# ZencashOfficial/ginger-lib

Hardware: AMD Instinct MI355X
Metric: MNT4-753 G1 MSM scalar-muls/sec + 2^n NTT ms at 1/2/4/8 MI355X (higher is better)
Workload: dtype u32 (29-bit limbs of 753-bit Montgomery residues, 64-bit accumulators)

## Files before the change

ginger-lib_amd/asmgen/build.py:

```python
import json
import os
import subprocess
import sys

from . import g1_reduce, g1_xyzz, g2_rounds, microbench, ntt_pass
from .isa import module_text

LLVM = os.environ.get("GH_LLVM_BIN", "/opt/rocm/lib/llvm/bin")

P4 = 0x1c4c62d92c41110229022eee2cdadb7f997505b8fafed5eb7e8f96c97d87307fdb925e8a0ed8d99d124d9a15af79db117e776f218059db80f0da5cb537e38685acce9767254a4638810719ac425f0e39d54522cdd119f5e9063de245e8001
P6 = 0x1c4c62d92c41110229022eee2cdadb7f997505b8fafed5eb7e8f96c97d87307fdb925e8a0ed8d99d124d9a15af79db26c5c28c859a99b3eebca9429212636b9dff97634993aa4d6c381bc3f0057974ea099170fa13a4fd90776e240000001
R = 1 << 754


def programs():
    progs = [
        g1_xyzz.build("gh_asm_acc_g1_p4", P4, R % P4),
        g1_xyzz.build("gh_asm_acc_g1_p6", P6, R % P6),
        g1_xyzz.build("gh_asm_acc_g1_p4_pw", P4, R % P4, persistent=True),
        g1_xyzz.build("gh_asm_acc_g1_p6_pw", P6, R % P6, persistent=True),
        g1_reduce.build("gh_asm_red_g1_p4", P4, R % P4),
        g1_reduce.build("gh_asm_red_g1_p6", P6, R % P6),
    ]
    c2 = g2_rounds.Cfg(2, 13, P4, R % P4)
# ... 6 lines not shown
                progs.append(g2_rounds.build("gh_asm_aff_%s_%s_%s" % (tag, "fwd" if fwd else "bwd", "r0" if r0 else "rn"), cfg, fwd, r0))
    for tag, prime in (("p4", P4), ("p6", P6)):
        for k in (6, 7, 8):
            progs.append(ntt_pass.build("gh_asm_ntt_%s_k%d" % (tag, k), prime, k))
    progs.append(microbench.build("gh_asm_mb_mulpair", P4))
    if os.environ.get("GH_ASM_DEBUG"):
        progs.append(g2_rounds.build("gh_asm_aff_f2_bwd_r0_dbg", c2, False, True, debug=True))
        for tag, prime in (("p4", P4), ("p6", P6)):
            progs.append(g1_xyzz.build("gh_asm_acc_g1_%s_dbg" % tag, prime, R % prime, debug=True))
            progs.append(g1_xyzz.build("gh_asm_acc_g1_%s_pw_dbg" % tag, prime, R % prime, persistent=True, debug=True))
    if os.environ.get("GH_ASM_VARIANTS"):
        progs += [g1_xyzz.build("gh_asm_acc_g1_p4_s1", P4, R % P4, split=1),
                  g1_xyzz.build("gh_asm_acc_g1_p4_s2", P4, R % P4, split=2),
                  g1_xyzz.build("gh_asm_acc_g1_p4_s1pf", P4, R % P4, split=1, prefetch=True)]
    return progs


def build(outdir):
    os.makedirs(outdir, exist_ok=True)
    progs = programs()
    text, infos = module_text(progs)
    s_path = os.path.join(outdir, "gh_asm.s")
    with open(s_path, "w") as f:
        f.write(text)
    o_path = os.path.join(outdir, "gh_asm.o")
    co_path = os.path.join(outdir, "gh_asm.hsaco")
    subprocess.run([os.path.join(LLVM, "clang"), "-x", "assembler", "-target", "amdgcn-amd-amdhsa", "-mcpu=gfx950",
                    "-c", s_path, "-o", o_path], check=True)
    subprocess.run([os.path.join(LLVM, "ld.lld"), "-shared", o_path, "-o", co_path], check=True)
    for p in progs:
        infos[p.name]["instructions"] = p.count()
        infos[p.name]["lds_bytes"] = p.lds_bytes
        infos[p.name]["scratch_bytes_per_lane"] = 0
    with open(os.path.join(outdir, "gh_asm.json"), "w") as f:
        json.dump(infos, f, indent=1, sort_keys=True)
    return co_path, infos


if __name__ == "__main__":
    co, infos = build(sys.argv[1] if len(sys.argv) > 1 else "build")
    print(co, json.dumps(infos))
```

ginger-lib_amd/asmgen/field.py:

```python
from .isa import Reg, V, S

NL = 26
LB = 29
LM = (1 << LB) - 1


def limbs(x, n=NL):
    return [(x >> (LB * i)) & LM for i in range(n)]


def unlimbs(l):
    return sum(int(v) << (LB * i) for i, v in enumerate(l))


class Chain:

    def __init__(self, acc, t0, t1, sdum, scar):
        self.acc = acc
        self.t0 = t0
        self.t1 = t1
        self.sdum = sdum
        self.scar = scar


class FieldGen:
    def __init__(self, prog, p, s_p, s_np, s_inv, s_lm):
        self.g = prog
        self.p = p
        self.pl = limbs(p)
        self.inv = (-pow(p, -1, 1 << LB)) % (1 << LB)
        self.s_p = s_p
        self.s_np = s_np
        self.s_inv = s_inv
        self.s_lm = s_lm

    def sP(self, i):
        return S(self.s_p + i)
# ... 227 lines not shown
                g.v_add3_u32(u, t, self.sNP(i), bw); yield
            g.v_ashrrev_i32(bw, LB, u); yield
            g.v_and_b32(b.sub(i), S(self.s_lm), u); yield
        g.v_cmp_eq_u32(ch.scar, 0, bw); yield
        for i in range(NL):
            g.v_cndmask_b32(a.sub(i), a.sub(i), b.sub(i), ch.scar); yield

    def neg_sel(self, ch, y, tmp, sel):
        g = self.g
        m, t0, lmm, x, c = ch.t1, ch.t0, ch.acc.lo(), ch.acc.hi(), tmp
        g.v_cndmask_b32(m, 0, -1, sel); yield
        g.v_and_b32(lmm, S(self.s_lm), m); yield
        g.v_and_b32(c, 1, m); yield
        for i in range(NL):
            g.v_and_b32(t0, self.sP(i), m); yield
            g.v_xor_b32(x, y.sub(i), lmm); yield
            g.v_add3_u32(x, x, t0, c); yield
            g.v_lshrrev_b32(c, LB, x); yield
            g.v_and_b32(y.sub(i), S(self.s_lm), x); yield

    def is_zero_mask(self, ch, a, smask):
        g = self.g
        t = ch.t0
        g.v_or3_b32(t, a.sub(0), a.sub(1), a.sub(2)); yield
        i = 3
        while i < NL:
            if i + 1 < NL:
                g.v_or3_b32(t, t, a.sub(i), a.sub(i + 1)); i += 2
            else:
                g.v_or_b32(t, t, a.sub(i)); i += 1
            yield
        g.v_cmp_eq_u32(smask, 0, t); yield

    def set_const(self, slot, value):
        for i, l in enumerate(limbs(value)):
            self.g.v_mov_b32(slot.sub(i), l)
            yield

    def copy(self, dst, src):
        for i in range(NL):
            self.g.v_mov_b32(dst.sub(i), src.sub(i))
            yield


def run(gen):
    for _ in gen:
        pass


def interleave(*gens):
    gens = list(gens)
    while gens:
        for g in list(gens):
            try:
                next(g)
            except StopIteration:
                gens.remove(g)
```

ginger-lib_amd/asmgen/g1_xyzz.py:

```python
from .isa import Prog, V, S, VCC, EXEC, OFF, fix_hazards
from .field import FieldGen, Chain, interleave, run, NL, LM

AFF_BYTES = 2 * NL * 4
PROJ_WORDS = 3 * NL
PARK_X, PARK_V, PARK_RR = 0, 1, 2
LDS_BYTES = 3 * NL * 256 * 4

S_KARG = S(0, 2)
S_WG = S(2)
S_BASES, S_SORTED, S_TASKS, S_SALTS = S(4, 2), S(6, 2), S(8, 2), S(10, 2)
S_NTASKS = S(12)
S_208 = S(13)
S_LM, S_INV = 20, 21
S_P, S_NP = 24, 50
S_ACTIVE = S(76, 2)
S_NEGSEL = S(78, 2)
S_T0, S_T1 = S(80, 2), S(82, 2)
S_LAUNCH = S(84, 2)
S_SAVE = S(86, 2)
S_DETOUR = S(88, 2)
S_T2 = S(90, 2)
S_ZERO = S(92, 2)
S_CTR = S(96, 2)
S_NTILES = S(98)
S_TILE = S(99)
S_BUDGET = S(3)
S_STAMPS = S(100, 2)
STAMP_BYTES = 64

V_TID, V_LDS = V(0), V(1)
V_CUR = V(2, 2)
V_LEFT, V_PHASE, V_SNEG, V_SALT = V(4), V(5), V(6), V(7)
V_DST = V(8, 2)
V_ADDR = V(10, 2)
# ... 9 lines not shown
V_ST0, V_ST1, V_STID, V_STOFF = V(30, 4), V(34, 4), V(26, 4), V(38)


def slot(i):
    return V(40 + NL * i, NL)


def seq(*gens):
    for gen in gens:
        run(gen)


E = [slot(i) for i in range(8)]


def build(name, p, one_mont, prefetch=False, split=4, persistent=False, debug=False):
    assert not (debug and prefetch)
    g = Prog(name)
    lanes = 64 if persistent else 256
    park_stride = lanes * 4
    g.lds_bytes = 3 * NL * park_stride
    for _ in range(4):
        g.add_arg(8, "ptr")
    g.add_arg(4, "val")
    if persistent:
        g.add_arg(4, "val")
        off_ctr = g.add_arg(8, "ptr")
        off_budget = g.add_arg(4, "val")
    if debug:
        off_stamps = g.add_arg(8, "ptr")
    f = FieldGen(g, p, S_P, S_NP, S_INV, S_LM)
    chA = Chain(V(248, 2), V(252), V(253), S(14, 2), S(16, 2))
    chB = Chain(V(250, 2), V(254), V(255), S(18, 2), S(22, 2))

    def park_addr(which, w):
        if which < 2:
            return V_LDS, (which * NL + w) * park_stride
        return V_LDS2, ((which - 2) * NL + w) * park_stride

    def park_put(which, sl):
        for w in range(NL):
            a, off = park_addr(which, w)
            g.ds_write_b32(a, sl.sub(w), offset=off)

    def park_get(which, sl):
        for w in range(NL):
            a, off = park_addr(which, w)
            g.ds_read_b32(sl.sub(w), a, offset=off)

    L_LOOP, L_INIT, L_INIT_RET, L_DETOUR, L_DET_RET, L_ADV, L_DONE, L_START = (
        g.uniq(s) for s in ("loop", "init", "init_ret", "detour", "det_ret", "adv", "done", "start"))
    S_JMP = S(94, 2)

    def stamp(dst):
        g.s_memtime(S_T0)
        g.s_memrealtime(S_T1)
        g.s_waitcnt(lgkmcnt=0)
        g.v_mov_b32(dst.sub(0), S_T0.lo()); g.v_mov_b32(dst.sub(1), S_T0.hi())
        g.v_mov_b32(dst.sub(2), S_T1.lo()); g.v_mov_b32(dst.sub(3), S_T1.hi())

    def stamp_store():
        stamp(V_ST1)
        g.s_getreg_b32(S_T0.lo(), "hwreg(HW_REG_HW_ID)")
        g.s_getreg_b32(S_T0.hi(), "hwreg(HW_REG_XCC_ID)")
        g.v_mov_b32(V_STID.sub(0), S_T0.lo()); g.v_mov_b32(V_STID.sub(1), S_T0.hi())
        g.v_mov_b32(V_STID.sub(3), S_LAUNCH.lo())
# ... 48 lines not shown
            g.v_lshrrev_b32(V_STID.sub(2), 6, V_T[0])
            g.v_lshlrev_b32(V_STOFF, 6, V_STID.sub(2))
        reset_task(V_T[0], with_constants=True)
        g.s_branch(L_LOOP)
    else:
        g.s_waitcnt(lgkmcnt=0)
        wave_constants()
        g.label(L_FETCH)
        g.s_mov_b64(EXEC, 1)
        g.v_mov_b32(V_T[0], 1)
        g.v_mov_b32(V_T[1], 0)
        g.global_atomic_add(V_T[2], V_T[1], V_T[0], S_CTR, sc0=True)
        g.s_waitcnt(vmcnt=0)
        g.v_readfirstlane_b32(S_TILE, V_T[2])
        g.s_mov_b64(EXEC, -1)
        g.s_cmp_ge_u32(S_TILE, S_NTILES)
        g.s_cbranch_scc1(L_EXIT)
        g.v_lshl_or_b32(V_T[0], S_TILE, 6, V_TID)
        g.v_cmp_gt_u32(VCC, S_NTASKS, V_T[0])
        g.s_and_b64(EXEC, EXEC, VCC)
        g.s_cbranch_execz(L_FETCH)
        g.s_mov_b64(S_LAUNCH, EXEC)
        if debug:
            stamp(V_ST0)
            g.v_mov_b32(V_STID.sub(2), S_TILE)
            g.v_lshlrev_b32(V_STOFF, 6, V_STID.sub(2))
        reset_task(V_T[0])
        g.s_branch(L_LOOP)
        g.label(L_EXIT)
        g.s_endpgm()

    g.label(L_DONE)
    g.s_mov_b64(EXEC, S_LAUNCH)
    run(f.is_zero_mask(chA, E[0], S_ZERO))
    park_get(PARK_X, E[2])
    park_get(PARK_V, E[3])
    g.v_cmp_ne_u32(S_NEGSEL, 0, V_SNEG)
    g.s_waitcnt(lgkmcnt=0)
    for w in range(NL):
        g.v_and_b32(E[2].sub(w), S(S_LM), E[2].sub(w))
        g.v_and_b32(E[3].sub(w), S(S_LM), E[3].sub(w))
    run(f.neg_sel(chA, E[3], V_TMP, S_NEGSEL))
    seq(f.mul(chA, E[2], E[1], E[4], E[2]),
        f.mul(chB, E[3], E[0], E[5], E[3]))
    run(f.cond_sub(chA, E[0], E[6], E[0]))
    run(f.mul(chA, E[0], E[1], E[6], E[2]))
    g.s_mov_b64(S_SAVE, EXEC)
    g.s_and_b64(EXEC, EXEC, S_ZERO)
    for w in range(NL):
        g.v_mov_b32(E[4].sub(w), 0)
        g.v_mov_b32(E[6].sub(w), 0)
    run(f.set_const(E[5], one_mont))
    g.s_mov_b64(EXEC, S_SAVE)
    for j in range(PROJ_WORDS // 2):
        g.global_store_dwordx2(V_DST, V(E[4].idx + 2 * j, 2), OFF, offset=8 * j)
    if debug:
        stamp_store()
    if persistent:
        g.s_sub_u32(S_BUDGET, S_BUDGET, 1)
        g.s_cmp_eq_u32(S_BUDGET, 0)
        g.s_cbranch_scc0(L_FETCH)
        g.s_endpgm()
    else:
        g.s_endpgm()

    g.label(L_LOOP)
    g.s_mov_b64(EXEC, S_LAUNCH)
    g.v_cmp_ne_u32(S_ACTIVE, 0, V_LEFT)
    g.v_cmp_ne_u32(S_T0, 0, V_GUARD)
    g.s_and_b64(S_ACTIVE, S_ACTIVE, S_T0)
    g.s_mov_b64(S_DETOUR, 0)
    g.s_and_b64(EXEC, S_ACTIVE, EXEC)
    g.s_cbranch_execz(L_DONE)
    g.global_load_dword(V_E, V_CUR, OFF)
    if prefetch:
        g.v_cmp_lt_u32(S_T1, 1, V_LEFT)
        g.v_cndmask_b32(V_T[2], 0, 4, S_T1)
        g.v_add_co_u32(V_NADDR.lo(), VCC, V_CUR.lo(), V_T[2])
        g.v_addc_co_u32(V_NADDR.hi(), VCC, 0, V_CUR.hi(), VCC)
        g.global_load_dword(V_ENEXT, V_NADDR, OFF)
    g.v_and_b32(V_T[1], 1, V_PHASE)
    g.v_cmp_ne_u32(S_T0, 0, V_T[1])
    g.v_mad_u64_u32(V(16, 2), chA.sdum, V_SALT, S_208, V_SALTS)
    g.s_waitcnt(vmcnt=0)
    g.v_and_b32(V_T[0], 0x7FFFFFFF, V_E)
    g.v_mad_u64_u32(V_ADDR, chA.sdum, V_T[0], S_208, V_BASES)
    g.v_cndmask_b32(V_ADDR.lo(), V_ADDR.lo(), V(16), S_T0)
    g.v_cndmask_b32(V_ADDR.hi(), V_ADDR.hi(), V(17), S_T0)
    if split > 1:
        g.s_mov_b64(S_SAVE, EXEC)
    for q in range(split):
        if split > 1:
            g.s_bfm_b64(S_T1, 64 // split, (64 // split) * q)
            g.s_and_b64(EXEC, S_SAVE, S_T1)
        for j in range(AFF_BYTES // 16):
            g.global_load_dwordx4(V(E[2].idx + 4 * j, 4), V_ADDR, OFF, offset=16 * j)
    if split > 1:
        g.s_mov_b64(EXEC, S_SAVE)
    g.v_lshrrev_b32(V_T[0], 31, V_E)
    g.v_lshrrev_b32(V_T[1], 1, V_PHASE)
    g.v_cndmask_b32(V_T[0], V_T[0], V_T[1], S_T0)
    g.v_xor_b32(V_T[0], V_T[0], V_SNEG)
    g.v_cmp_ne_u32(S_NEGSEL, 0, V_T[0])
    g.s_waitcnt(vmcnt=0)
    if prefetch:
        g.v_and_b32(V_T[2], 0x7FFFFFFF, V_ENEXT)
        g.v_mad_u64_u32(V_NADDR, chA.sdum, V_T[2], S_208, V_BASES)
        for j in range(4):
            g.global_load_dword(V_TOUCH, V_NADDR, OFF, offset=min(64 * j, AFF_BYTES - 4))
    run(f.neg_sel(chA, E[3], V_TMP, S_NEGSEL))
    run(f.is_zero_mask(chA, E[0], S_ZERO))
    g.s_cmp_lg_u64(S_ZERO, 0)
    g.s_cbranch_scc0(L_INIT_RET)
    g.long_branch(L_INIT, S_JMP)
    g.label(L_INIT_RET)

    seq(f.mul(chA, E[2], E[0], E[4], E[2]),
        f.mul(chB, E[3], E[1], E[5], E[3]))
    park_get(PARK_X, E[2])
    park_get(PARK_V, E[3])
    g.s_waitcnt(lgkmcnt=0)
    interleave(f.sub(chA, E[4], E[2], E[4]),
               f.sub(chB, E[5], E[3], E[5]))
    interleave(f.is_zero_mask(chA, E[4], S_T0), f.is_zero_mask(chB, E[5], S_T1))
    g.v_cmp_eq_u32(S_T2, 0, V_PHASE)
    g.s_and_b64(S_T0, S_T0, S_T1)
    g.s_and_b64(S_DETOUR, S_T0, S_T2)
    g.s_cbranch_scc0(L_DET_RET)
    g.long_branch(L_DETOUR, S_JMP)
    g.label(L_DET_RET)
    seq(f.sqr(chA, E[4], E[2], E[6]),
        f.sqr(chB, E[5], E[3], E[7]))
    park_put(PARK_RR, E[7])
    seq(f.mul(chA, E[4], E[6], E[2], E[4], dst=E[4]),
        f.mul(chB, E[0], E[6], E[3], E[0], dst=E[0], reduce=False))
    park_get(PARK_X, E[2])
    g.s_waitcnt(lgkmcnt=0)
    seq(f.mul(chA, E[2], E[6], E[3], E[2], dst=E[2]),
        f.mul(chB, E[1], E[4], E[7], E[1], dst=E[1], reduce=False))
    park_get(PARK_RR, E[3])
    g.s_waitcnt(lgkmcnt=0)
    run(f.sub(chA, E[3], E[4], E[3]))
    run(f.sub(chA, E[3], E[2], E[3]))
    run(f.sub(chA, E[3], E[2], E[3]))
    park_put(PARK_X, E[3])
    park_get(PARK_V, E[6])
    run(f.sub(chA, E[3], E[2], E[2]))
    g.s_waitcnt(lgkmcnt=0)
    run(f.dual(chA, chB, E[5], E[2], E[6], E[4], E[7], E[6]))
    park_put(PARK_V, E[7])
    g.v_xor_b32(V_SNEG, 1, V_SNEG)

    g.label(L_ADV)
    g.s_andn2_b64(EXEC, S_ACTIVE, S_DETOUR)
    g.v_cmp_eq_u32(S_T0, 0, V_PHASE)
    g.v_cmp_eq_u32(S_T1, 3, V_PHASE)
    g.s_or_b64(S_T0, S_T0, S_T1)
    g.v_add_u32(V_T[0], 1, V_PHASE)
    g.v_cndmask_b32(V_PHASE, V_T[0], 0, S_T0)
    g.v_cndmask_b32(V_T[0], 0, 1, S_T0)
    g.v_sub_u32(V_LEFT, V_LEFT, V_T[0])
    g.v_lshlrev_b32(V_T[0], 2, V_T[0])
    g.v_add_co_u32(V_CUR.lo(), VCC, V_CUR.lo(), V_T[0])
    g.v_addc_co_u32(V_CUR.hi(), VCC, 0, V_CUR.hi(), VCC)
    g.s_mov_b64(EXEC, S_ACTIVE)
    g.v_subrev_u32(V_GUARD, 1, V_GUARD)
    g.long_branch(L_LOOP, S_JMP)

    g.label(L_INIT)
    g.s_mov_b64(S_SAVE, EXEC)
    g.s_mov_b64(EXEC, S_ZERO)
    park_put(PARK_X, E[2])
    park_put(PARK_V, E[3])
    run(f.set_const(E[0], one_mont))
    run(f.set_const(E[1], one_mont))
    g.s_andn2_b64(EXEC, S_SAVE, S_ZERO)
    g.s_cbranch_execz(L_ADV)
    g.long_branch(L_INIT_RET, S_JMP)

    g.label(L_DETOUR)
    g.s_mov_b64(S_SAVE, EXEC)
    g.s_mov_b64(EXEC, S_DETOUR)
    for j in range(NL // 2):
        g.global_load_dwordx2(V(E[2].idx + 2 * j, 2), V_ADDR, OFF, offset=8 * j)
    for j in range(NL // 2):
        g.global_load_dwordx2(V(E[3].idx + 2 * j, 2), V_SALTS, OFF, offset=8 * j)
    g.s_waitcnt(vmcnt=0)
    for w in range(NL):
        g.v_xor_b32(E[2].sub(w), E[2].sub(w), E[3].sub(w))
    run(f.is_zero_mask(chA, E[2], S_T0))
    g.v_cndmask_b32(V_SALT, 0, 1, S_T0)
    g.v_mov_b32(V_PHASE, 1)
    g.s_andn2_b64(EXEC, S_SAVE, S_DETOUR)
    g.s_cbranch_execz(L_ADV)
    g.long_branch(L_DET_RET, S_JMP)
    g.hazard_nops = fix_hazards(g)
    return g
```

ginger-lib_amd/asmgen/sim.py:

```python
import numpy as np

from .isa import Reg

U32 = np.uint32
U64 = np.uint64
M32 = 0xFFFFFFFF
LANES = 64
_AR = np.arange(LANES, dtype=U64)


def mask_arr(m):
    return ((U64(m) >> _AR) & U64(1)).astype(bool)


def arr_mask(a):
    return int(np.packbits(a.astype(np.uint8), bitorder="little").view(U64)[0])


class MemFault(Exception):
    pass


class Memory:

# ... 33 lines not shown

    def store(self, addr, vals):
        if addr & 3:
            raise MemFault("unaligned store 0x%x" % addr)
        arr, i = self._find(addr, 4 * len(vals), True)
        self.stores += 1
        arr[i:i + len(vals)] = vals


class Wave:
    def __init__(self, prog, mem, lds_words=0):
        self.prog = prog
        self.mem = mem
        self.V = np.zeros((512, LANES), dtype=U32)
        self.S = [0] * 128
        self.scc = 0
        self.lds = np.zeros(max(lds_words, 1), dtype=U32)
        self.labels = {}
        for n, i in enumerate(prog.ins):
            if i.op == "label":
                self.labels[i.args[0]] = n
        self.executed = 0
        self.hist = {}
        self.set_exec((1 << 64) - 1)

    def set_exec(self, m):
        self.S[126] = m & M32
        self.S[127] = (m >> 32) & M32

    def exec_mask(self):
        return self.S[126] | (self.S[127] << 32)

    def em(self):
        return mask_arr(self.exec_mask())

    def ridx(self, r):
        k = r.kind
        if k == "v":
            return r.idx
        if k == "a":
            return 256 + r.idx
        raise TypeError(r)

    def rd(self, o):
        if isinstance(o, Reg):
            if o.kind in ("v", "a"):
                assert o.n == 1, o
                return self.V[self.ridx(o)]
            assert o.n == 1 or o.kind in ("vcc", "exec"), o
            return U32(self.S[o.idx])
        return U32(o & M32)

    def rd64(self, o):
        if isinstance(o, Reg):
            if o.kind in ("v", "a"):
                assert o.n == 2, o
                i = self.ridx(o)
                return self.V[i].astype(U64) | (self.V[i + 1].astype(U64) << U64(32))
            assert o.n == 2, o
            return U64(self.S[o.idx] | (self.S[o.idx + 1] << 32))
        return U64(o & 0xFFFFFFFFFFFFFFFF)

    def rd_smask(self, o):
        assert isinstance(o, Reg) and o.n == 2 and o.kind in ("s", "vcc", "exec"), o
        return self.S[o.idx] | (self.S[o.idx + 1] << 32)

    def wr_smask(self, o, m):
# ... 14 lines not shown
        i = self.ridx(o)
        self.V[i][em] = (val & U64(M32)).astype(U32)[em]
        self.V[i + 1][em] = (val >> U64(32)).astype(U32)[em]

    def wr_lanemask(self, o, arr):
        self.wr_smask(o, arr_mask(np.asarray(arr, dtype=bool) & self.em()))

    def ws(self, o, val):
        assert isinstance(o, Reg) and o.kind == "s" and o.n == 1, o
        self.S[o.idx] = int(val) & M32

    def rs(self, o):
        if isinstance(o, Reg):
            assert o.n == 1 and o.kind in ("s",), o
            return self.S[o.idx]
        return o & M32

    def _check_inflight(self, i):
        op = i.op
        if op == "s_waitcnt":
            if "vmcnt" in i.mods and getattr(self, "_inflight_vm", None) is not None:
                keep = int(i.mods["vmcnt"])
                self._vm_fifo = self._vm_fifo[len(self._vm_fifo) - keep:] if keep else []
                self._inflight_vm = set().union(*self._vm_fifo) if self._vm_fifo else set()
            if i.mods.get("lgkmcnt") == 0:
                self._inflight_lgkm = set()
            return
        vm = getattr(self, "_inflight_vm", None)
        if vm is None:
            vm = self._inflight_vm = set()
            self._inflight_lgkm = set()
            self._vm_fifo = []
        lg = self._inflight_lgkm
        regs = set()
        for a in i.args:
            if isinstance(a, Reg) and a.kind in ("v", "a"):
                base = a.idx + (256 if a.kind == "a" else 0)
                regs.update(range(base, base + a.n))
            elif isinstance(a, Reg) and a.kind == "s":
                regs.update(-1 - r for r in range(a.idx, a.idx + a.n))
        own = set()
        if op.startswith("global_load") and isinstance(i.args[0], Reg):
            d0 = i.args[0]
            own = set(range(d0.idx, d0.idx + d0.n)) & vm
        hit = (regs - own) & (vm | lg)
        if hit:
            raise RuntimeError("%s touches a register with a result in flight (no s_waitcnt): %s" % (
                i.text().strip(), sorted(("v%d" % r) if r >= 0 else ("s%d" % (-1 - r)) for r in hit)[:6]))
        dst = None
        if op.startswith("global_load") or (op.startswith("global_atomic") and i.mods.get("sc0")):
            dst, pend = i.args[0], vm
        elif op.startswith("ds_read") or op in ("ds_bpermute_b32", "ds_permute_b32", "ds_swizzle_b32"):
            dst, pend = i.args[0], lg
        elif op.startswith("s_load"):
            dst, pend = i.args[0], lg
        if op.startswith("global_store") or (op.startswith("global_atomic") and not i.mods.get("sc0")):
            self._vm_fifo.append(set())
        if dst is not None:
            if dst.kind in ("v", "a"):
                base = dst.idx + (256 if dst.kind == "a" else 0)
                pend.update(range(base, base + dst.n))
                if pend is vm:
                    self._vm_fifo.append(set(range(base, base + dst.n)))
            else:
                pend.update(-1 - r for r in range(dst.idx, dst.idx + dst.n))

# ... 699 lines not shown
```

ginger-lib_amd/csrc/ec29.h:

```cpp
#pragma once
#include "fp29.h"

namespace gh {

struct Mnt4G1 {
    typedef P4 PF;
    typedef F1<P4, true> F;
    typedef F1<P4, false> FC;
    static GH_HD F::T mul_by_a(const F::T& z) { return fp_dbl<P4>(z); }
};
struct Mnt6G1 {
    typedef P6 PF;
    typedef F1<P6, true> F;
    typedef F1<P6, false> FC;
    static GH_HD F::T mul_by_a(const F::T& z) { return fp_mul_small<P6, 11>(z); }
};
struct Mnt4G2 {
    typedef P4 PF;
    typedef F2<P4, 13, false> F;
    typedef F2<P4, 13, false> FC;
    static GH_HD F::T mul_by_a(const F::T& z) { return F::T{fp_mul_small<P4, 26>(z.c0), fp_mul_small<P4, 26>(z.c1)}; }
};
struct Mnt6G2 {
    typedef P6 PF;
// ... 82 lines not shown
template <class C> GH_HD_NOINLINE Proj<C> proj_madd_call(const Proj<C>& p, const Aff<C>& q) { return proj_madd<C, typename C::FC>(p, q); }

template <class C> GH_HD Aff<C> aff_neg(const Aff<C>& q) { return Aff<C>{q.x, C::F::neg(q.y)}; }

template <class C> struct Xyzz {
    typename C::F::T x, y, zz, zzz;
};
template <class C> GH_HD Xyzz<C> xyzz_zero() {
    typedef typename C::F F;
    return Xyzz<C>{F::zero(), F::one(), F::zero(), F::zero()};
}
template <class C> GH_HD bool xyzz_is_zero(const Xyzz<C>& p) { return C::F::is_zero(p.zz); }
template <class C, class F = typename C::F> GH_HD Xyzz<C> xyzz_madd(const Xyzz<C>& p, const Aff<C>& q, bool& same) {
    same = false;
    if (xyzz_is_zero(p)) return Xyzz<C>{q.x, q.y, F::one(), F::one()};
    typename F::T pp = F::sub(F::mul(q.x, p.zz), p.x);
    typename F::T r = F::sub(F::mul(q.y, p.zzz), p.y);
    if (F::is_zero(pp) && F::is_zero(r)) { same = true; return p; }
    typename F::T p2 = F::sqr(pp);
    typename F::T p3 = F::mul(pp, p2);
    typename F::T qq = F::mul(p.x, p2);
    Xyzz<C> o;
    o.x = F::sub(F::sub(F::sqr(r), p3), F::dbl(qq));
    o.y = F::mul_sub_mul(r, F::sub(qq, o.x), p.y, p3);
    o.zz = F::mul(p.zz, p2);
    o.zzz = F::mul(p.zzz, p3);
    return o;
}
template <class C, class F = typename C::F> GH_HD Proj<C> xyzz_to_proj(const Xyzz<C>& p) {
    if (xyzz_is_zero(p)) return proj_zero<C>();
    return Proj<C>{F::mul(p.x, p.zzz), F::mul(p.y, p.zz), F::mul(p.zz, p.zzz)};
}

}
```

ginger-lib_amd/csrc/fp29.h:

```cpp
#pragma once
#include <stdint.h>
#include "constants_gen.h"

#if defined(__HIPCC__)
#define GH_HD __host__ __device__ __forceinline__
#define GH_HD_NOINLINE __host__ __device__ __attribute__((noinline))
#define GH_UNROLL _Pragma("unroll")
#else
#define GH_HD inline
#define GH_HD_NOINLINE __attribute__((noinline))
#define GH_UNROLL
#endif

namespace gh {

constexpr int NL = 26;
constexpr int LB = 29;
constexpr uint32_t LM = (1u << LB) - 1;

struct Fp {
    uint32_t l[NL];
};

struct P4 {
// ... 230 lines not shown
            int32_t x = (int32_t)r.l[i] - (int32_t)P::P[i] + bw;
            dd[i] = (uint32_t)x & LM;
            bw = x >> 31;
        }
        const bool take = top != 0 || bw == 0;
        GH_UNROLL for (int i = 0; i < NL; i++) r.l[i] = take ? dd[i] : r.l[i];
    }
    fp_cond_sub<P>(r);
    return r;
}

template <class P> GH_HD Fp fp_sqr(const Fp& a) {
    uint32_t m[NL], a2[NL];
    Fp r;
    GH_UNROLL for (int i = 0; i < NL; i++) a2[i] = a.l[i] << 1;
    uint64_t acc = 0;
    GH_UNROLL for (int k = 0; k < NL; k++) {
        GH_UNROLL for (int i = 0; 2 * i < k; i++) acc += (uint64_t)a.l[i] * a2[k - i];
        if ((k & 1) == 0) acc += (uint64_t)a.l[k / 2] * a.l[k / 2];
        GH_UNROLL for (int i = 0; i < k; i++) acc += (uint64_t)m[i] * P::P[k - i];
        m[k] = ((uint32_t)acc * P::INV) & LM;
        acc += (uint64_t)m[k] * P::P[0];
        acc >>= LB;
    }
    GH_UNROLL for (int k = NL; k < 2 * NL; k++) {
        GH_UNROLL for (int i = k - NL + 1; 2 * i < k; i++) acc += (uint64_t)a.l[i] * a2[k - i];
        if ((k & 1) == 0) acc += (uint64_t)a.l[k / 2] * a.l[k / 2];
        GH_UNROLL for (int i = k - NL + 1; i < NL; i++) acc += (uint64_t)m[i] * P::P[k - i];
        r.l[k - NL] = (uint32_t)acc & LM;
        acc >>= LB;
    }
    fp_cond_sub<P>(r);
    return r;
}

constexpr int FP_INV_BATCHES = 61;

template <class P> GH_HD Fp fp_inv_plain(const Fp& x) {
    int32_t d[NL], e[NL], f[NL], g[NL];
    GH_UNROLL for (int i = 0; i < NL; i++) { d[i] = 0; e[i] = 0; f[i] = (int32_t)P::P[i]; g[i] = (int32_t)x.l[i]; }
    e[0] = 1;
    int32_t zeta = -1;
    const uint32_t pinv = (0u - P::INV) & LM;
#if defined(__HIP_DEVICE_COMPILE__)
#pragma nounroll
#endif
    for (int it = 0; it < FP_INV_BATCHES; it++) {
        uint32_t u = 1, v = 0, q = 0, r = 1, fl = (uint32_t)f[0], gl = (uint32_t)g[0];
#if defined(__HIP_DEVICE_COMPILE__)
#pragma nounroll
#endif
        for (int s = 0; s < LB; s++) {
            uint32_t m1 = (uint32_t)(zeta >> 31);
            const uint32_t m2 = 0u - (gl & 1u);
            const uint32_t xf = (fl ^ m1) - m1, yu = (u ^ m1) - m1, zv = (v ^ m1) - m1;
            gl += xf & m2; q += yu & m2; r += zv & m2;
            m1 &= m2;
            zeta = (int32_t)((uint32_t)zeta ^ m1) - 1;
            fl += gl & m1; u += q & m1; v += r & m1;
            gl >>= 1; u <<= 1; v <<= 1;
        }
        const int64_t U = (int32_t)u, V = (int32_t)v, Q = (int32_t)q, R = (int32_t)r;
        {
            const int32_t sd = d[NL - 1] >> 31, se = e[NL - 1] >> 31;
            int32_t md = ((int32_t)U & sd) + ((int32_t)V & se), me = ((int32_t)Q & sd) + ((int32_t)R & se);
            int64_t cd = U * d[0] + V * e[0], ce = Q * d[0] + R * e[0];
// ... 226 lines not shown
```

Before: 56.56 million.

## Use lazy-reduction 27-digit Montgomery arithmetic in the G1 XYZZ bucket accumulator

Replaces the fully reduced Montgomery mul/sqr/sub in the assembly XYZZ mixed-add loop with 27-digit Montgomery products that skip the final conditional subtraction. It also adds lazy differences that add a multiple of p instead of branching on borrow. Bounds are tracked per operand at generation time, and zero tests become zero-or-p tests. The aim is to cut VALU work per bucket update by dropping cond_subs and reductions, at the cost of one extra Montgomery digit per product and an extra normalising multiply and cond_subs at the end. A C++ reference implementation and simulator speedups come along with it.

Measured after the change: 57.94 million (median of 6 runs). 1.02x the previous value.

```diff
diff --git a/ginger-lib_amd/asmgen/build.py b/ginger-lib_amd/asmgen/build.py
--- a/ginger-lib_amd/asmgen/build.py
+++ b/ginger-lib_amd/asmgen/build.py
@@ -62,6 +62,8 @@
         infos[p.name]["instructions"] = p.count()
         infos[p.name]["lds_bytes"] = p.lds_bytes
         infos[p.name]["scratch_bytes_per_lane"] = 0
+        if getattr(p, "loop_labels", None):
+            infos[p.name].update(g1_xyzz.update_counts(p))
     with open(os.path.join(outdir, "gh_asm.json"), "w") as f:
         json.dump(infos, f, indent=1, sort_keys=True)
     return co_path, infos
diff --git a/ginger-lib_amd/asmgen/field.py b/ginger-lib_amd/asmgen/field.py
--- a/ginger-lib_amd/asmgen/field.py
+++ b/ginger-lib_amd/asmgen/field.py
@@ -3,6 +3,34 @@
 NL = 26
 LB = 29
 LM = (1 << LB) - 1
+
+
+ND = NL + 1
+TOP_SHIFT = LB * (NL - 1)
+
+
+class BoundError(ValueError):
+    """a lazy routine was asked for operands whose columns, top limb or doubled limb do not fit the registers"""
+
+
+class Bound:
+
+    def __init__(self, k, slack=0):
+        self.k, self.slack = k, slack
+
+    def value(self, p):
+        return self.k * p + self.slack
+
+    def __repr__(self):
+        return "Bound(%d p + 2^%.1f)" % (self.k, _log2(self.slack)) if self.slack else "Bound(%d p)" % self.k
+
+
+def _bound(b):
+    return b if isinstance(b, Bound) else Bound(*b) if isinstance(b, tuple) else Bound(b)
+
+
+def _log2(x):
+    return x.bit_length() - 1 + (x >> max(0, x.bit_length() - 53)) / (1 << min(52, x.bit_length() - 1)) - 1 if x > 0 else 0.0
 
 
 def limbs(x, n=NL):
@@ -296,6 +324,165 @@
             yield
         g.v_cmp_eq_u32(smask, 0, t); yield
 
+    def _caps(self, bd):
+        top = _bound(bd).value(self.p) >> TOP_SHIFT
+        if top >> 32:
+            raise BoundError("top limb of an operand can reach 2^32 (bound %r)" % (bd,))
+        return [LM] * (NL - 1) + [top]
+
+    def _md(self, ch, m, i):
+        return m.sub(i) if i < NL else ch.t1
+
+    def plan27(self, groups, value_sum, allow_split=True):
+        split, carry = set(), 0
+        for k in range(2 * NL):
+            sums = [sum(cap for _, _, cap in terms(k)) for terms in groups]
+            mp = sum(LM * self.pl[k - i] for i in range(max(0, k - NL + 1), min(k, ND - 1) + 1))
+            total = carry + sum(sums) + mp
+            if total >> 64 == 0:
+                carry = total >> LB
+                continue
+            part1, part2 = carry + sums[0], LM + sum(sums[1:]) + mp
+            if len(groups) < 2 or not allow_split or part1 >> 64 or part2 >> 64:
+                raise BoundError("column %d of a 27-digit product can reach 2^%.2f" % (k, _log2(total)))
+            split.add(k)
+            carry = (part1 >> LB) + (part2 >> LB)
+        res = Bound(1, value_sum >> (LB * ND))
+        self._caps(res)
+        return split, res
+
+    def mont_columns27(self, ch, groups, split, m, r, ch2=None):
+        g = self.g
+        X = ch.acc
+        first = True
+        for k in range(2 * NL):
+            acc = X
+            for n, terms in enumerate(groups):
+                if n == 1 and k in split:
+                    acc = ch2.acc
+                    g.v_and_b32(acc.lo(), S(self.s_lm), X.lo()); yield
+                    g.v_mov_b32(acc.hi(), 0); yield
+                    g.v_lshrrev_b64(X, LB, X); yield
+                for (x, y, _) in terms(k):
+                    g.v_mad_u64_u32(acc, ch.sdum, x, y, 0 if first else acc); first = False; yield
+            for i in range(max(0, k - NL + 1), min(k - 1, ND - 1) + 1):
+                g.v_mad_u64_u32(acc, ch.sdum, self._md(ch, m, i), self.sP(k - i), acc); yield
+            if k < ND:
+                mk = self._md(ch, m, k)
+                g.v_mul_lo_u32(ch.t0, acc.lo(), S(self.s_inv)); yield
+                g.v_and_b32(mk, S(self.s_lm), ch.t0); yield
+                g.v_mad_u64_u32(acc, ch.sdum, mk, self.sP(0), acc); yield
+                g.v_lshrrev_b64(acc, LB, acc); yield
+            elif k < 2 * NL - 1:
+                g.v_and_b32(r.sub(k - ND), S(self.s_lm), acc.lo()); yield
+                g.v_lshrrev_b64(acc, LB, acc); yield
+            else:
+                assert acc is X
+                g.v_and_b32(r.sub(NL - 2), S(self.s_lm), X.lo()); yield
+                g.v_alignbit_b32(r.sub(NL - 1), X.hi(), X.lo(), LB); yield
+            if acc is not X:
+                g.v_lshl_add_u64(X, acc, 0, X); yield
+
+    def _terms27(self, a, b, ca, cb):
+        def terms(k):
+            return [(a.sub(i), b.sub(k - i), ca[i] * cb[k - i]) for i in range(max(0, k - NL + 1), min(k, NL - 1) + 1)]
+        return terms
+
+    def mul27(self, ch, a, b, m, ba, bb, r=None):
+        ba, bb = _bound(ba), _bound(bb)
+        groups = [self._terms27(a, b, self._caps(ba), self._caps(bb))]
+        split, res = self.plan27(groups, ba.value(self.p) * bb.value(self.p))
+        yield from self.mont_columns27(ch, groups, split, m, m if r is None else r)
+        return res
+
+    def sqr27(self, ch, a, a2, m, ba, r=None):
+        ba = _bound(ba)
+        ca = self._caps(ba)
+        if (2 * ca[NL - 1]) >> 32:
+            raise BoundError("doubled top limb of a squaring operand can reach 2^32 (bound %r)" % (ba,))
+
+        def terms(k):
+            t = [(a.sub(i), a2.sub(k - i), 2 * ca[i] * ca[k - i]) for i in range(max(0, k - NL + 1), NL) if 2 * i < k and k - i < NL]
+            if k % 2 == 0 and k // 2 < NL:
+                t.append((a.sub(k // 2), a.sub(k // 2), ca[k // 2] ** 2))
+            return t
+        split, res = self.plan27([terms], ba.value(self.p) ** 2)
+        for i in range(NL):
+            self.g.v_lshlrev_b32(a2.sub(i), 1, a.sub(i)); yield
+        yield from self.mont_columns27(ch, [terms], split, m, m if r is None else r)
+        return res
+
+    def dual27(self, ch, ch2, a, b, c, d, m, ba, bb, bc, bd, r=None, allow_split=True):
+        ba, bb, bc, bd = (_bound(x) for x in (ba, bb, bc, bd))
+        groups = [self._terms27(a, b, self._caps(ba), self._caps(bb)), self._terms27(c, d, self._caps(bc), self._caps(bd))]
+        split, res = self.plan27(groups, ba.value(self.p) * bb.value(self.p) + bc.value(self.p) * bd.value(self.p), allow_split)
+        self.last_split = sorted(split)
+        yield from self.mont_columns27(ch, groups, split, m, m if r is None else r, ch2)
+        return res
+
+    def lazy_diff(self, ch, a, subs, s, dst, ba, bsubs):
+        g = self.g
+        ba = Bound(0) if a is None else _bound(ba)
+        bsubs = [_bound(x) for x in bsubs]
+        kp = self.p << s
+        K = limbs(kp, NL - 1) + [kp >> TOP_SHIFT]
+        ca = self._caps(ba)
+        cs = [self._caps(x) for x in bsubs]
+        low = sum(mult * x.value(self.p) for (_, mult), x in zip(subs, bsubs))
+        if low > kp:
+            raise BoundError("a lazy difference can be negative: subtrahends up to %.2f p against %d p" % (low / self.p, 1 << s))
+        res = Bound(ba.k + (1 << s), ba.slack)
+        self._caps(res)
+        cmin = cmax = 0
+        for i in range(NL):
+            hi = ca[i] + K[i] + cmax
+            lo = cmin - sum(mult * c[i] for (_, mult), c in zip(subs, cs))
+            if i + 1 < NL and (hi >> 31 or lo < -(1 << 31)):
+                raise BoundError("limb %d of a lazy difference leaves 32 signed bits" % i)
+            cmin, cmax = lo >> LB, hi >> LB
+        t, x, c = ch.t0, ch.acc.lo(), ch.t1
+        for i in range(NL):
+            if len(subs) == 1:
+                (b, mult), = subs
+                assert mult == 1
+                g.v_sub_u32(t, K[i], b.sub(i)); yield
+            else:
+                (b, mb), (q, mq) = subs
+                assert (mb, mq) == (1, 2)
+                g.v_lshl_add_u32(t, q.sub(i), 1, b.sub(i)); yield
+                g.v_sub_u32(t, K[i], t); yield
+            o = dst.sub(i) if i == NL - 1 else x
+            if a is None:
+                if i:
+                    g.v_add_u32(o, t, c); yield
+                else:
+                    g.v_mov_b32(o, t); yield
+            elif i:
+                g.v_add3_u32(o, t, a.sub(i), c); yield
+            else:
+                g.v_add_u32(o, t, a.sub(0)); yield
+            if i + 1 < NL:
+                g.v_ashrrev_i32(c, LB, x); yield
+                g.v_and_b32(dst.sub(i), S(self.s_lm), x); yield
+        return res
+
+    def zero_or_p_mask(self, ch, a, smask, stmp):
+        g = self.g
+        skip = g.uniq("zp_skip")
+        g.v_cmp_eq_u32(smask, 0, a.sub(0))
+        g.v_cmp_eq_u32(stmp, self.sP(0), a.sub(0))
+        g.s_or_b64(smask, smask, stmp)
+        g.s_cbranch_scc0(skip)
+        run(self.is_zero_mask(ch, a, smask))
+        x = ch.acc.lo()
+        g.v_xor_b32(x, self.sP(0), a.sub(0))
+        for i in range(1, NL):
+            g.v_xor_b32(ch.t1, self.sP(i), a.sub(i))
+            g.v_or_b32(x, x, ch.t1)
+        g.v_cmp_eq_u32(stmp, 0, x)
+        g.s_or_b64(smask, smask, stmp)
+        g.label(skip)
+
     def set_const(self, slot, value):
         for i, l in enumerate(limbs(value)):
             self.g.v_mov_b32(slot.sub(i), l)
@@ -310,6 +497,14 @@
 def run(gen):
     for _ in gen:
         pass
+
+
+def runv(gen):
+    while True:
+        try:
+            next(gen)
+        except StopIteration as e:
+            return e.value
 
 
 def interleave(*gens):
diff --git a/ginger-lib_amd/asmgen/g1_xyzz.py b/ginger-lib_amd/asmgen/g1_xyzz.py
--- a/ginger-lib_amd/asmgen/g1_xyzz.py
+++ b/ginger-lib_amd/asmgen/g1_xyzz.py
@@ -1,5 +1,5 @@
 from .isa import Prog, V, S, VCC, EXEC, OFF, fix_hazards
-from .field import FieldGen, Chain, interleave, run, NL, LM
+from .field import FieldGen, Chain, Bound, run, runv, NL, LB
 
 AFF_BYTES = 2 * NL * 4
 PROJ_WORDS = 3 * NL
@@ -75,6 +75,17 @@
     f = FieldGen(g, p, S_P, S_NP, S_INV, S_LM)
     chA = Chain(V(248, 2), V(252), V(253), S(14, 2), S(16, 2))
     chB = Chain(V(250, 2), V(254), V(255), S(18, 2), S(22, 2))
+    c_lazy = one_mont * (1 << (2 * LB)) % p
+    AR = Bound(1, 1 << 733)
+    B_TAB = Bound(1)
+    B_X = Bound(5, 1 << 733)
+
+    def within(b, decl):
+        assert b.value(p) <= decl.value(p), (b, decl)
+        return decl
+
+    def mul27(ch, a, b, m, ba, bb, r=None, decl=AR):
+        return within(runv(f.mul27(ch, a, b, m, ba, bb, r)), decl)
 
     def park_addr(which, w):
         if which < 2:
@@ -189,19 +200,22 @@
 
     g.label(L_DONE)
     g.s_mov_b64(EXEC, S_LAUNCH)
-    run(f.is_zero_mask(chA, E[0], S_ZERO))
+    f.zero_or_p_mask(chA, E[0], S_ZERO, S_T0)
     park_get(PARK_X, E[2])
     park_get(PARK_V, E[3])
     g.v_cmp_ne_u32(S_NEGSEL, 0, V_SNEG)
     g.s_waitcnt(lgkmcnt=0)
+    b_neg = runv(f.lazy_diff(chA, None, [(E[3], 1)], 1, E[4], None, [AR]))
     for w in range(NL):
-        g.v_and_b32(E[2].sub(w), S(S_LM), E[2].sub(w))
-        g.v_and_b32(E[3].sub(w), S(S_LM), E[3].sub(w))
-    run(f.neg_sel(chA, E[3], V_TMP, S_NEGSEL))
-    seq(f.mul(chA, E[2], E[1], E[4], E[2]),
-        f.mul(chB, E[3], E[0], E[5], E[3]))
-    run(f.cond_sub(chA, E[0], E[6], E[0]))
-    run(f.mul(chA, E[0], E[1], E[6], E[2]))
+        g.v_cndmask_b32(E[3].sub(w), E[3].sub(w), E[4].sub(w), S_NEGSEL)
+    mul27(chA, E[2], E[1], E[4], B_X, AR)
+    mul27(chB, E[3], E[0], E[5], b_neg, AR)
+    mul27(chA, E[0], E[1], E[6], AR, AR)
+    run(f.set_const(E[7], one_mont))
+    mul27(chA, E[6], E[7], E[2], AR, B_TAB, r=E[6])
+    run(f.cond_sub(chA, E[4], E[2], E[4]))
+    run(f.cond_sub(chA, E[5], E[2], E[5]))
+    run(f.cond_sub(chA, E[6], E[2], E[6]))
     g.s_mov_b64(S_SAVE, EXEC)
     g.s_and_b64(EXEC, EXEC, S_ZERO)
     for w in range(NL):
@@ -266,45 +280,45 @@
         for j in range(4):
             g.global_load_dword(V_TOUCH, V_NADDR, OFF, offset=min(64 * j, AFF_BYTES - 4))
     run(f.neg_sel(chA, E[3], V_TMP, S_NEGSEL))
-    run(f.is_zero_mask(chA, E[0], S_ZERO))
+    f.zero_or_p_mask(chA, E[0], S_ZERO, S_T0)
     g.s_cmp_lg_u64(S_ZERO, 0)
     g.s_cbranch_scc0(L_INIT_RET)
     g.long_branch(L_INIT, S_JMP)
     g.label(L_INIT_RET)
 
-    seq(f.mul(chA, E[2], E[0], E[4], E[2]),
-        f.mul(chB, E[3], E[1], E[5], E[3]))
+    mul27(chA, E[2], E[0], E[4], B_TAB, AR)
+    mul27(chB, E[3], E[1], E[5], B_TAB, AR)
     park_get(PARK_X, E[2])
     park_get(PARK_V, E[3])
     g.s_waitcnt(lgkmcnt=0)
-    interleave(f.sub(chA, E[4], E[2], E[4]),
-               f.sub(chB, E[5], E[3], E[5]))
-    interleave(f.is_zero_mask(chA, E[4], S_T0), f.is_zero_mask(chB, E[5], S_T1))
+    b_p = runv(f.lazy_diff(chA, E[4], [(E[2], 1)], 3, E[4], AR, [B_X]))
+    b_w = runv(f.lazy_diff(chB, E[5], [(E[3], 1)], 1, E[5], AR, [AR]))
+    within(runv(f.sqr27(chA, E[4], E[2], E[6], b_p)), AR)
+    within(runv(f.sqr27(chB, E[5], E[3], E[7], b_w)), AR)
+    f.zero_or_p_mask(chA, E[6], S_T0, S_T2)
+    f.zero_or_p_mask(chB, E[7], S_T1, S_T2)
     g.v_cmp_eq_u32(S_T2, 0, V_PHASE)
     g.s_and_b64(S_T0, S_T0, S_T1)
     g.s_and_b64(S_DETOUR, S_T0, S_T2)
     g.s_cbranch_scc0(L_DET_RET)
     g.long_branch(L_DETOUR, S_JMP)
     g.label(L_DET_RET)
-    seq(f.sqr(chA, E[4], E[2], E[6]),
-        f.sqr(chB, E[5], E[3], E[7]))
     park_put(PARK_RR, E[7])
-    seq(f.mul(chA, E[4], E[6], E[2], E[4], dst=E[4]),
-        f.mul(chB, E[0], E[6], E[3], E[0], dst=E[0], reduce=False))
+    mul27(chA, E[4], E[6], E[2], b_p, AR, r=E[4])
+    mul27(chB, E[0], E[6], E[3], AR, AR, r=E[0])
     park_get(PARK_X, E[2])
     g.s_waitcnt(lgkmcnt=0)
-    seq(f.mul(chA, E[2], E[6], E[3], E[2], dst=E[2]),
-        f.mul(chB, E[1], E[4], E[7], E[1], dst=E[1], reduce=False))
+    mul27(chA, E[2], E[6], E[3], B_X, AR, r=E[2])
+    mul27(chB, E[1], E[4], E[7], AR, AR, r=E[1])
     park_get(PARK_RR, E[3])
     g.s_waitcnt(lgkmcnt=0)
-    run(f.sub(chA, E[3], E[4], E[3]))
-    run(f.sub(chA, E[3], E[2], E[3]))
-    run(f.sub(chA, E[3], E[2], E[3]))
+    within(runv(f.lazy_diff(chA, E[3], [(E[4], 1), (E[2], 2)], 2, E[3], AR, [AR, AR])), B_X)
     park_put(PARK_X, E[3])
     park_get(PARK_V, E[6])
-    run(f.sub(chA, E[3], E[2], E[2]))
-    g.s_waitcnt(lgkmcnt=0)
-    run(f.dual(chA, chB, E[5], E[2], E[6], E[4], E[7], E[6]))
+    b_t = runv(f.lazy_diff(chA, E[3], [(E[2], 1)], 1, E[2], B_X, [AR]))
+    g.s_waitcnt(lgkmcnt=0)
+    within(runv(f.dual27(chA, chB, E[5], E[2], E[6], E[4], E[7], b_w, b_t, AR, AR)), AR)
+    g.dual_split = f.last_split
     park_put(PARK_V, E[7])
     g.v_xor_b32(V_SNEG, 1, V_SNEG)
 
@@ -327,10 +341,12 @@
     g.label(L_INIT)
     g.s_mov_b64(S_SAVE, EXEC)
     g.s_mov_b64(EXEC, S_ZERO)
-    park_put(PARK_X, E[2])
-    park_put(PARK_V, E[3])
-    run(f.set_const(E[0], one_mont))
-    run(f.set_const(E[1], one_mont))
+    run(f.set_const(E[0], c_lazy))
+    run(f.set_const(E[1], c_lazy))
+    mul27(chA, E[2], E[0], E[4], B_TAB, B_TAB)
+    mul27(chB, E[3], E[0], E[5], B_TAB, B_TAB)
+    park_put(PARK_X, E[4])
+    park_put(PARK_V, E[5])
     g.s_andn2_b64(EXEC, S_SAVE, S_ZERO)
     g.s_cbranch_execz(L_ADV)
     g.long_branch(L_INIT_RET, S_JMP)
@@ -352,4 +368,25 @@
     g.s_cbranch_execz(L_ADV)
     g.long_branch(L_DET_RET, S_JMP)
     g.hazard_nops = fix_hazards(g)
+    g.loop_labels = (L_LOOP, L_ADV)
     return g
+
+
+def update_counts(g):
+    at = {i.args[0]: n for n, i in enumerate(g.ins) if i.op == "label"}
+    n, end = at[g.loop_labels[0]], None
+    total = valu = mads = 0
+    while end is None:
+        i = g.ins[n]
+        n += 1
+        if i.op in ("label", "comment"):
+            continue
+        total += 1
+        valu += i.op.startswith("v_")
+        mads += i.op == "v_mad_u64_u32"
+        if i.op == "s_cbranch_scc0" and at[i.args[0]] > n:
+            n = at[i.args[0]]
+        elif i.op == "long_branch":
+            assert i.args[0] == g.loop_labels[0]
+            end = n
+    return dict(update_instructions=total, update_valu=valu, update_mads=mads)
diff --git a/ginger-lib_amd/asmgen/sim.py b/ginger-lib_amd/asmgen/sim.py
--- a/ginger-lib_amd/asmgen/sim.py
+++ b/ginger-lib_amd/asmgen/sim.py
@@ -89,7 +89,11 @@
         return self.S[126] | (self.S[127] << 32)
 
     def em(self):
-        return mask_arr(self.exec_mask())
+        m = self.exec_mask()
+        if m != getattr(self, "_em_key", None):
+            self._em_key, self._em = m, mask_arr(m)
+            self._em.setflags(write=False)
+        return self._em
 
     def ridx(self, r):
         k = r.kind
@@ -170,6 +174,8 @@
             self._inflight_lgkm = set()
             self._vm_fifo = []
         lg = self._inflight_lgkm
+        if not vm and not lg and not op.startswith(("global_", "ds_", "s_load")):
+            return
         regs = set()
         for a in i.args:
             if isinstance(a, Reg) and a.kind in ("v", "a"):
diff --git a/ginger-lib_amd/csrc/ec29.h b/ginger-lib_amd/csrc/ec29.h
--- a/ginger-lib_amd/csrc/ec29.h
+++ b/ginger-lib_amd/csrc/ec29.h
@@ -138,4 +138,51 @@
     return Proj<C>{F::mul(p.x, p.zzz), F::mul(p.y, p.zz), F::mul(p.zz, p.zzz)};
 }
 
+struct XyzzLazy {
+    Fp x, v, zz, zzz;
+    uint32_t sneg;
+};
+GH_HD XyzzLazy xyzz_lazy_zero() { return XyzzLazy{fp_zero(), fp_zero(), fp_zero(), fp_zero(), 0u}; }
+template <class P> GH_HD bool xyzz_lazy_is_zero(const XyzzLazy& s) { return fp_is_zero_or_p<P>(s.zz); }
+template <class P> GH_HD void xyzz_madd_lazy(XyzzLazy& s, const Fp& qx, const Fp& qy_row, bool neg, bool& same) {
+    same = false;
+    const Fp qy = (neg != (s.sneg != 0)) ? fp_neg_lazy<P>(qy_row) : qy_row;
+    if (xyzz_lazy_is_zero<P>(s)) {
+        const Fp c = fp_lazy_one<P>();
+        s.x = fp_mul27<P>(qx, c);
+        s.v = fp_mul27<P>(qy, c);
+        s.zz = c;
+        s.zzz = c;
+        return;
+    }
+    const Fp pp = fp_lazy_sub<P, 3>(fp_mul27<P>(qx, s.zz), s.x);
+    const Fp w = fp_lazy_sub<P, 1>(fp_mul27<P>(qy, s.zzz), s.v);
+    const Fp p2 = fp_sqr27<P>(pp);
+    const Fp rr = fp_sqr27<P>(w);
+    if (fp_is_zero_or_p<P>(p2) && fp_is_zero_or_p<P>(rr)) { same = true; return; }
+    const Fp p3 = fp_mul27<P>(pp, p2);
+    const Fp q = fp_mul27<P>(s.x, p2);
+    s.zz = fp_mul27<P>(s.zz, p2);
+    s.zzz = fp_mul27<P>(s.zzz, p3);
+    s.x = fp_lazy_x3<P>(rr, p3, q);
+    const Fp t = fp_lazy_sub<P, 1>(s.x, q);
+    s.v = fp_mul2s27<P>(w, t, s.v, p3);
+    s.sneg ^= 1u;
 }
+template <class P> GH_HD void xyzz_lazy_to_proj(const XyzzLazy& s, Fp& x, Fp& y, Fp& z) {
+    if (xyzz_lazy_is_zero<P>(s)) {
+        x = fp_zero();
+        y = fp_one<P>();
+        z = fp_zero();
+        return;
+    }
+    const Fp yy = s.sneg ? fp_lazy_sub<P, 1>(fp_zero(), s.v) : s.v;
+    x = fp_mul27<P>(s.x, s.zzz);
+    y = fp_mul27<P>(yy, s.zz);
+    z = fp_mul27<P>(fp_mul27<P>(s.zz, s.zzz), fp_one<P>());
+    fp_cond_sub<P>(x);
+    fp_cond_sub<P>(y);
+    fp_cond_sub<P>(z);
+}
+
+}
diff --git a/ginger-lib_amd/csrc/fp29.h b/ginger-lib_amd/csrc/fp29.h
--- a/ginger-lib_amd/csrc/fp29.h
+++ b/ginger-lib_amd/csrc/fp29.h
@@ -286,6 +286,128 @@
     }
     fp_cond_sub<P>(r);
     return r;
+}
+
+constexpr int ND = NL + 1;
+template <class P> struct Dual27Split;
+template <> struct Dual27Split<P4> { static constexpr uint64_t MASK = (1ull << 25) | (1ull << 26); };
+template <> struct Dual27Split<P6> { static constexpr uint64_t MASK = 1ull << 25; };
+
+template <class P> GH_HD Fp fp_mul27(const Fp& a, const Fp& b) {
+    uint32_t m[ND];
+    Fp r;
+    uint64_t acc = 0;
+    GH_UNROLL for (int k = 0; k < 2 * NL; k++) {
+        GH_UNROLL for (int i = (k < NL ? 0 : k - NL + 1); i <= (k < NL ? k : NL - 1); i++) acc += (uint64_t)a.l[i] * b.l[k - i];
+        GH_UNROLL for (int i = (k < NL ? 0 : k - NL + 1); i <= (k <= ND ? k - 1 : ND - 1); i++) acc += (uint64_t)m[i] * P::P[k - i];
+        if (k < ND) {
+            m[k] = ((uint32_t)acc * P::INV) & LM;
+            acc += (uint64_t)m[k] * P::P[0];
+        } else {
+            r.l[k - ND] = (uint32_t)acc & LM;
+        }
+        acc >>= LB;
+    }
+    r.l[NL - 1] = (uint32_t)acc;
+    return r;
+}
+
+template <class P> GH_HD Fp fp_sqr27(const Fp& a) {
+    uint32_t m[ND], a2[NL];
+    Fp r;
+    GH_UNROLL for (int i = 0; i < NL; i++) a2[i] = a.l[i] << 1;
+    uint64_t acc = 0;
+    GH_UNROLL for (int k = 0; k < 2 * NL; k++) {
+        GH_UNROLL for (int i = (k < NL ? 0 : k - NL + 1); 2 * i < k; i++) acc += (uint64_t)a.l[i] * a2[k - i];
+        if ((k & 1) == 0 && k / 2 < NL) acc += (uint64_t)a.l[k / 2] * a.l[k / 2];
+        GH_UNROLL for (int i = (k < NL ? 0 : k - NL + 1); i <= (k <= ND ? k - 1 : ND - 1); i++) acc += (uint64_t)m[i] * P::P[k - i];
+        if (k < ND) {
+            m[k] = ((uint32_t)acc * P::INV) & LM;
+            acc += (uint64_t)m[k] * P::P[0];
+        } else {
+            r.l[k - ND] = (uint32_t)acc & LM;
+        }
+        acc >>= LB;
+    }
+    r.l[NL - 1] = (uint32_t)acc;
+    return r;
+}
+
+template <class P, uint64_t SPLIT = Dual27Split<P>::MASK> GH_HD Fp fp_mul2s27(const Fp& a, const Fp& b, const Fp& c, const Fp& d) {
+    uint32_t m[ND];
+    Fp r;
+    uint64_t acc = 0;
+    GH_UNROLL for (int k = 0; k < 2 * NL; k++) {
+        const bool split = (SPLIT >> k) & 1;
+        GH_UNROLL for (int i = (k < NL ? 0 : k - NL + 1); i <= (k < NL ? k : NL - 1); i++) acc += (uint64_t)a.l[i] * b.l[k - i];
+        uint64_t keep = 0;
+        if (split) {
+            keep = acc >> LB;
+            acc &= LM;
+        }
+        GH_UNROLL for (int i = (k < NL ? 0 : k - NL + 1); i <= (k < NL ? k : NL - 1); i++) acc += (uint64_t)c.l[i] * d.l[k - i];
+        GH_UNROLL for (int i = (k < NL ? 0 : k - NL + 1); i <= (k <= ND ? k - 1 : ND - 1); i++) acc += (uint64_t)m[i] * P::P[k - i];
+        if (k < ND) {
+            m[k] = ((uint32_t)acc * P::INV) & LM;
+            acc += (uint64_t)m[k] * P::P[0];
+        } else {
+            r.l[k - ND] = (uint32_t)acc & LM;
+        }
+        acc = (acc >> LB) + keep;
+    }
+    r.l[NL - 1] = (uint32_t)acc;
+    return r;
+}
+
+template <class P, int S> GH_HD uint32_t fp_kp_limb(int i) {
+    const uint32_t lo = i ? P::P[i - 1] >> (LB - S) : 0u;
+    return (i == NL - 1 ? P::P[i] << S : (P::P[i] << S) & LM) + lo;
+}
+template <class P, int S> GH_HD Fp fp_lazy_sub(const Fp& a, const Fp& b) {
+    Fp t;
+    int32_t cy = 0;
+    GH_UNROLL for (int i = 0; i < NL; i++) {
+        const uint32_t x = fp_kp_limb<P, S>(i) - b.l[i] + a.l[i] + (uint32_t)cy;
+        t.l[i] = i == NL - 1 ? x : x & LM;
+        cy = (int32_t)x >> LB;
+    }
+    return t;
+}
+template <class P> GH_HD Fp fp_lazy_x3(const Fp& rr, const Fp& ppp, const Fp& q) {
+    Fp t;
+    int32_t cy = 0;
+    GH_UNROLL for (int i = 0; i < NL; i++) {
+        const uint32_t x = fp_kp_limb<P, 2>(i) - ((q.l[i] << 1) + ppp.l[i]) + rr.l[i] + (uint32_t)cy;
+        t.l[i] = i == NL - 1 ? x : x & LM;
+        cy = (int32_t)x >> LB;
+    }
+    return t;
+}
+template <class P> GH_HD Fp fp_neg_lazy(const Fp& y) {
+    Fp t;
+    int32_t bw = 0;
+    GH_UNROLL for (int i = 0; i < NL; i++) {
+        const int32_t x = (int32_t)P::P[i] - (int32_t)y.l[i] + bw;
+        t.l[i] = (uint32_t)x & LM;
+        bw = x >> 31;
+    }
+    return t;
+}
+template <class P> GH_HD bool fp_is_zero_or_p(const Fp& a) {
+    if (a.l[0] != 0 && a.l[0] != P::P[0]) return false;
+    uint32_t z = 0, e = 0;
+    GH_UNROLL for (int i = 0; i < NL; i++) {
+        z |= a.l[i];
+        e |= a.l[i] ^ P::P[i];
+    }
+    return z == 0 || e == 0;
+}
+template <class P> GH_HD Fp fp_lazy_one() {
+    Fp d3 = fp_zero();
+    d3.l[3] = 1;
+    Fp c = fp_mul27<P>(fp_const<P>(P::R2I), d3);
+    fp_cond_sub<P>(c);
+    return c;
 }
 
 constexpr int FP_INV_BATCHES = 61;
```
